# little-little-point-cloud-group/buildingSegment

Measured on AMD Instinct MI355X. Metric: Mpoints/s segmented (kNN+normal+label), higher is better.
Workload: dtype int32 coordinates / f64 normals; 1 GPU; urban_50m; points_per_gpu=50000000, k=16, max_nn=50, rg_mode=0, largest_plane=135921, seed_attempts=6951, fallback_queries=0, rg_rounds=25, validation_rejects=2, tie_rows=971975, parallelism=1 GPU, whole path

## Files before the change

### buildingsegment_amd/csrc/bs_grow_spec.hip

```cpp
#include <hipcub/hipcub.hpp>

#include <algorithm>
#include <cstdio>
#include <cstdlib>
#include <type_traits>
#include <chrono>
#include <vector>

#include "bs_centerdiv.h"
#include "bs_common.h"

namespace bs {

namespace {

constexpr int32_t INF = 0x7fffffff;
constexpr int32_t LOWER_BIT = (int32_t)0x80000000;
constexpr int32_t POS_MASK = 0x7fffffff;
constexpr int MAX_WAVES = 1 << 18;
constexpr int MAX_PENDING = 32768;

enum : int32_t { ST_NONE = 0, ST_DONE = 1, ST_FAILED0 = 2, ST_NOMEM = 3, ST_WATCHDOG = 4, ST_STOLEN = 5 };

struct SpecArgs {
// ... 188 lines not shown
    lcnt[d] = 0;
  __syncthreads();
  const uint32_t m0 = i < n ? hmask[i] : 0u;
  const uint32_t lm0 = i < n ? lmask[i] : 0u;
  const int32_t* row = rows + (i < n ? i : 0) * row_stride;
  for (uint32_t m = m0; m;) {
    const int t = __ffs(m) - 1;
    m &= m - 1;
    const int64_t d = (int64_t)row[t + 1] - w0;
    if (d >= 0 && d < RW_WIN)
      atomicAdd(&lcnt[d], 1);
  }
  __syncthreads();
  for (int d = threadIdx.x; d < RW_WIN; d += 256) {
    const int v = lcnt[d];
    if (v) {
      lbase[d] = atomicAdd(&rcur[w0 + d], (unsigned long long)v);
      lcnt[d] = 0;
    }
  }
  __syncthreads();
  for (uint32_t m = m0; m;) {
    const int t = __ffs(m) - 1;
    m &= m - 1;
    const int32_t c = row[t + 1];
    const int64_t d = (int64_t)c - w0;
    if (d >= 0 && d < RW_WIN)
      radj[lbase[d] + (unsigned)atomicAdd(&lcnt[d], 1)] = (int32_t)i | (((lm0 >> t) & 1u) ? LOWER_BIT : 0);
    else
      radj[atomicAdd(&rcur[c], 1ull)] = (int32_t)i | (((lm0 >> t) & 1u) ? LOWER_BIT : 0);
  }
}

__global__ void pull_pass_kernel(int64_t n, int K, int sub, const uint32_t* __restrict__ hmask,
                                 const int32_t* __restrict__ prio, const uint8_t* __restrict__ ps,
                                 const int32_t* __restrict__ base, const int64_t* __restrict__ roff,
                                 const int32_t* __restrict__ radj, int32_t* __restrict__ omega, uint32_t* occ,
                                 uint8_t* dirty_cur, uint8_t* dirty_next, uint8_t* bdirty_cur, uint8_t* bdirty_next,
                                 int4* rec, int quads, int* any, const int32_t* __restrict__ minr, const int* prev_any)
{
  if (prev_any && *prev_any == 0)
    return;
  __shared__ unsigned long long sub_mask;
  const int64_t nb256 = (n + 255) >> 8;
  const int64_t g0 = (int64_t)blockIdx.x * sub;
  if (threadIdx.x < 64) {
    const int64_t gidx = g0 + threadIdx.x;
    const bool d = (int)threadIdx.x < sub && gidx < nb256 && bdirty_cur[gidx] != 0;
    if (d)
      bdirty_cur[gidx] = 0;
    const unsigned long long m = ballot64(d);
    if (threadIdx.x == 0)
      sub_mask = m;
  }
  __syncthreads();
  unsigned long long gm = sub_mask;
  bool flipped = false;
  while (gm) {
    const int t = __ffsll(gm) - 1;
    gm &= gm - 1;
    const int64_t c = ((g0 + t) << 8) + threadIdx.x;
    if (c >= n || !dirty_cur[c])
      continue;
    dirty_cur[c] = 0;
    int32_t v = base[c];
    if (v > minr[c]) {
      const int64_t e1 = roff[c + 1];
      for (int64_t e = roff[c]; e < e1; e += 4) {
        int32_t j[4];
        uint32_t ow[4];
        int32_t pj[4];
#pragma unroll
        for (int i = 0; i < 4; i++)
          j[i] = e + i < e1 ? (radj[e + i] & POS_MASK) : -1;
#pragma unroll
        for (int i = 0; i < 4; i++)
          ow[i] = j[i] >= 0 ? __hip_atomic_load(occ + (j[i] >> 5), __ATOMIC_RELAXED, __HIP_MEMORY_SCOPE_AGENT) : 0u;
#pragma unroll
        for (int i = 0; i < 4; i++)
          pj[i] = ((ow[i] >> (j[i] & 31)) & 1u) ? prio[j[i]] : INF;
#pragma unroll
        for (int i = 0; i < 4; i++)
          v = pj[i] < v ? pj[i] : v;
      }
    }
    omega[c] = v;
    reinterpret_cast<int32_t*>(rec + c * quads)[3] = v;
    const uint32_t m0 = hmask[c];
    const uint8_t want = (m0 != 0 && !(ps[c] & 1) && v >= prio[c]) ? 1 : 0;
    const uint32_t cbit = 1u << (c & 31);
    const uint8_t have = (__hip_atomic_load(occ + (c >> 5), __ATOMIC_RELAXED, __HIP_MEMORY_SCOPE_AGENT) & cbit) ? 1 : 0;
    if (want != have) {
      if (want)
        __hip_atomic_fetch_or(occ + (c >> 5), cbit, __ATOMIC_RELAXED, __HIP_MEMORY_SCOPE_AGENT);
      else
        __hip_atomic_fetch_and(occ + (c >> 5), ~cbit, __ATOMIC_RELAXED, __HIP_MEMORY_SCOPE_AGENT);
      const int32_t* row = reinterpret_cast<const int32_t*>(rec + c * quads + 4);
      uint32_t m = m0;
      while (m) {
        const int b = __ffs(m) - 1;
        m &= m - 1;
        const int32_t q = row[b + 1];
        dirty_next[q] = 1;
        bdirty_next[q >> 8] = 1;
      }
      flipped = true;
    }
  }
  if (flipped)
    *any = 1;
}

__global__ void decide_init_kernel(const uint32_t* __restrict__ hmask, int64_t n, uint8_t* __restrict__ st,
                                   uint8_t* __restrict__ bund)
{
  const int64_t c = blockIdx.x * (int64_t)blockDim.x + threadIdx.x;
  const bool maker = c < n && hmask[c] != 0;
  if (c < n)
    st[c] = maker ? 0 : 2;
  const int anym = __syncthreads_or(maker);
  if (threadIdx.x == 0)
    bund[blockIdx.x] = anym ? 1 : 0;
}

__global__ void decide_pass_kernel(int64_t n, int sub, const int32_t* __restrict__ prio,
                                   const int64_t* __restrict__ roff, const int32_t* __restrict__ radj, uint8_t* st,
                                   uint8_t* bund, int* any)
{
  __shared__ unsigned long long sub_mask;
  __shared__ int left[64];
  const int64_t nb256 = (n + 255) >> 8;
  const int64_t g0 = (int64_t)blockIdx.x * sub;
  if (threadIdx.x < 64) {
    const int64_t gidx = g0 + threadIdx.x;
    const bool d = (int)threadIdx.x < sub && gidx < nb256 && bund[gidx] != 0;
    left[threadIdx.x] = 0;
    const unsigned long long m = ballot64(d);
    if (threadIdx.x == 0)
      sub_mask = m;
  }
  __syncthreads();
  unsigned long long gm = sub_mask;
  bool undecided_left = false;
  while (gm) {
    const int t = __ffsll(gm) - 1;
    gm &= gm - 1;
    const int64_t c = ((g0 + t) << 8) + threadIdx.x;
    bool mine_left = false;
    if (c < n && __hip_atomic_load(st + c, __ATOMIC_RELAXED, __HIP_MEMORY_SCOPE_AGENT) == 0) {
      bool lower_occ = false, lower_und = false;
      const int64_t e1 = roff[c + 1];
      for (int64_t e = roff[c]; e < e1; e += 4) {
        int32_t rj[4];
        uint8_t sj[4];
#pragma unroll
        for (int q = 0; q < 4; q++)
          rj[q] = e + q < e1 ? radj[e + q] : 0;
#pragma unroll
        for (int q = 0; q < 4; q++)
          sj[q] = rj[q] < 0 ? __hip_atomic_load(st + (rj[q] & POS_MASK), __ATOMIC_RELAXED, __HIP_MEMORY_SCOPE_AGENT) : (uint8_t)2;
#pragma unroll
// ... 82 lines not shown

__global__ void cand_flag_kernel(const int4* __restrict__ rec, int quads, int K,
                                 int64_t n, int32_t F, const int32_t* __restrict__ prio, const uint8_t* __restrict__ ps,
                                 int all_seeds, const int32_t* __restrict__ omega, int32_t* min_idx,
                                 unsigned long long* __restrict__ cand_out, int32_t* cand_count, uint8_t* __restrict__ bcand,
                                 int sub)
{
  __shared__ unsigned long long sub_mask;
  const int64_t nb256 = (n + 255) >> 8;
  const int64_t g0 = (int64_t)blockIdx.x * sub;
  if (threadIdx.x < 64) {
    const int64_t gidx = g0 + threadIdx.x;
    const bool live = (int)threadIdx.x < sub && gidx < nb256 && bcand[gidx] != 0;
    const unsigned long long m = ballot64(live);
    if (threadIdx.x == 0)
      sub_mask = m;
  }
  __syncthreads();
  unsigned long long gm = sub_mask;
  while (gm) {
    const int t = __ffsll(gm) - 1;
    gm &= gm - 1;
    const int64_t i = ((g0 + t) << 8) + threadIdx.x;
    bool c = false, alive = false;
    const uint8_t f = i < n ? ps[i] : (uint8_t)2;
    int32_t pi = 0;
    if (!(f & 2)) {
      pi = prio[i];
      const int32_t oi = omega[i];
      alive = !(oi < F);
      if (pi >= F && oi >= pi && (all_seeds || !(f & 1))) {
        c = true;
        const int32_t* row = reinterpret_cast<const int32_t*>(rec + i * quads + 4);
        for (int u = 1; u < K; u += 4) {
          int32_t ov[4];
#pragma unroll
          for (int q = 0; q < 4; q++)
            ov[q] = u + q < K ? omega[row[u + q]] : INF;
#pragma unroll
          for (int q = 0; q < 4; q++)
            c = c && ov[q] >= pi;
        }
      }
    }
    const int any_alive = __syncthreads_or(alive);
    if (threadIdx.x == 0 && !any_alive)
      bcand[g0 + t] = 0;
    if (c && min_idx)
      atomicMin(min_idx, pi);
    if (c && cand_out)
      cand_out[atomicAdd(cand_count, 1)] = ((unsigned long long)(uint32_t)pi << 32) | (uint32_t)i;
  }
}

template <int KC>
struct RecLayout {
  static constexpr int QUADS = 4 + KC / 4;
};

__device__ inline int32_t* rec_tag(int4* rec, int quads, int64_t i)
{
  return reinterpret_cast<int32_t*>(rec + i * quads + 2) + 2;
}

__global__ void invert_order_kernel(const int32_t* __restrict__ order, int64_t n, int32_t* __restrict__ pos)
{
  const int64_t s = blockIdx.x * (int64_t)blockDim.x + threadIdx.x;
  if (s < n)
    pos[order[s]] = (int32_t)s;
}

template <int KC>
__global__ __launch_bounds__(256) void build_records_kernel(SpecArgs a, const int32_t* __restrict__ order, const int32_t* __restrict__ pos,
// ... 1469 lines not shown
  gc = bs_grow_counters{};
  int retry_max_list = RETRY_MAX_LIST;
  bool retry_env = false;
  if (const char* e = getenv("BS_RETRY_MAX_LIST")) {
    retry_max_list = atoi(e);
    retry_env = true;
  }
  if (lim.retry_max_list >= 0) {
    retry_max_list = lim.retry_max_list;
    retry_env = true;
  }
  int retry_big_round = 1024;
  if (const char* e = getenv("BS_RETRY_BIG_ROUND"))
    retry_big_round = atoi(e);
  if (lim.retry_big_round >= 0)
    retry_big_round = lim.retry_big_round;
  int max_waves = MAX_WAVES;
  if (const char* e = getenv("BS_MAX_WAVES"))
    max_waves = atoi(e);
  if (lim.max_waves > 0)
    max_waves = (int)std::min<int64_t>(lim.max_waves, MAX_WAVES);
  const int wave_cap = (int)std::max<int64_t>(1, std::min<int64_t>(MAX_WAVES, n / 8 + 64));
  max_waves = (int)std::max<int64_t>(1, std::min<int64_t>(max_waves, wave_cap));
  const unsigned long long pool_cap = (unsigned long long)std::max<int64_t>(
      std::min<int64_t>(64 * n, (int64_t)3 << 30), 8 * n + (int64_t)(2 * 256 + 32 * 32) * 2 * wave_cap);
  const unsigned long long pool_cap_eff = lim.pool_cap > 0 ? std::min<unsigned long long>(pool_cap, (unsigned long long)lim.pool_cap) : pool_cap;
  gc.pool_cap = (int64_t)pool_cap_eff;
  gc.max_waves_end = max_waves;
  BS_HIP(ctx, ctx->rg_list.reserve(sizeof(int32_t) * list_cap));
  BS_HIP(ctx, ctx->rg_planes.reserve(sizeof(PlaneRec) * planes_cap));
  BS_HIP(ctx, ctx->rg_stats.reserve(sizeof(GrowStats)));
  const size_t n_i32 = (size_t)(7 * n + planes_cap + 1024 + 128);
  const size_t nb256 = (size_t)((n + 255) / 256);
  const size_t aux_bytes = sizeof(int32_t) * n_i32 + (size_t)5 * n + 3 * nb256 + 8192 +
                           sizeof(PlaneOut) * ((size_t)wave_cap + MAX_PENDING) +
                           sizeof(CopyDesc) * ((size_t)wave_cap + MAX_PENDING);
  BS_HIP(ctx, ctx->rg_aux.reserve(aux_bytes));
  BS_HIP(ctx, ctx->rg_stack.reserve(sizeof(int32_t) * pool_cap));
  BS_HIP(ctx, ctx->rg_radj.reserve(sizeof(int32_t) * (size_t)(n * (K - 1) + 16)));
  BS_HIP(ctx, ctx->rg_roff.reserve(sizeof(int64_t) * (size_t)(n + 2)));
  int64_t* roff = ctx->rg_roff.as<int64_t>();
  int32_t* aux = ctx->rg_aux.as<int32_t>();
  int32_t* d_misc = aux;
  uint32_t* hmask = (uint32_t*)(aux + 1024);
  int32_t* omega = aux + 1024 + n;
  int32_t* base = aux + 1024 + 2 * n;
  int32_t* dead = aux + 1024 + 3 * n;
  int32_t* prio = aux + 1024 + 4 * n;
  int32_t* rpos = aux + 1024 + 5 * n;
  int32_t* vmark = aux + 1024 + 6 * n + 64;
  int32_t* d_seeds = aux + 1024 + 7 * n + 64;
  uint8_t* flags = (uint8_t*)(aux + n_i32);
  uint8_t* ps = flags + n;
  uint32_t* occ = (uint32_t*)(((uintptr_t)(ps + n) + 15) & ~(uintptr_t)15);
  uint8_t* dirty0 = (uint8_t*)occ + ((n + 31) / 32) * 4 + 16;
  uint8_t* dirty1 = dirty0 + n;
  uint8_t* bdirty0 = dirty1 + n;
  uint8_t* bdirty1 = bdirty0 + nb256;
  uint8_t* bcand = bdirty1 + nb256;
  PlaneOut* d_out = (PlaneOut*)(((uintptr_t)(bcand + nb256) + 255) & ~(uintptr_t)255);
  PlaneOut* d_pend = d_out + wave_cap;
  CopyDesc* d_copy = (CopyDesc*)(d_pend + MAX_PENDING);
  int32_t* radj = ctx->rg_radj.as<int32_t>();
  unsigned long long* d_pool_top = (unsigned long long*)(d_misc + 16);
  Pool pool = {ctx->rg_stack.as<int32_t>(), d_pool_top, pool_cap_eff};

  SpecArgs a;
  a.xyz = d_xyz;
  a.normals = d_normals;
  a.neigh = d_neigh;
  a.n = n;
  a.K = K;
  a.th = (double)p.th_thickness;
  a.cos_th = p.cos_th;
  a.th_count = p.th_point_count;
  a.F = 0;
  a.pad = 0;

  const int KC = K <= 16 ? 16 : 32;
  const int quads = 4 + KC / 4;
  BS_HIP(ctx, ctx->rg_rec.reserve(sizeof(int4) * (size_t)quads * n));
  int4* rec = ctx->rg_rec.as<int4>();
  BS_HIP(ctx, ctx->rg_geo.reserve(sizeof(unsigned long long) * 2 * (size_t)(n + 64)));
  unsigned long long* cand_raw = ctx->rg_geo.as<unsigned long long>();
  BS_HIP(ctx, ctx->rg_gs.reserve(sizeof(int4) * 3 * (size_t)(n + 1)));
  int4* gs = ctx->rg_gs.as<int4>();
  unsigned long long* d_cand = cand_raw + n + 64;
  const size_t nt1 = (size_t)(n >> TILE1) + 2, nt2 = (size_t)(n >> TILE2) + 2;
  BS_HIP(ctx, ctx->rg_disp.reserve(sizeof(unsigned long long) * (nt1 + nt2) + sizeof(uint32_t) * 2 * (size_t)wave_cap + 64 +
                                    sizeof(PlaneOut) * (size_t)wave_cap));
  unsigned long long* tmin1 = ctx->rg_disp.as<unsigned long long>();
  unsigned long long* tmin2 = tmin1 + nt1;
  uint32_t* dkeys_in = reinterpret_cast<uint32_t*>(tmin2 + nt2);
// ... 16 lines not shown
  }
  const int4* spts_in = npos ? ctx->spts.as<int4>() : nullptr;
  const double* pnorm_in = (npos && ctx->npos_normals == d_normals) ? pnorm_of(ctx->seg_npos.as<int32_t>(), n, K) : nullptr;
  if (order && !npos) {
    pos = vmark;
    invert_order_kernel<<<nblk(n, 256), 256, 0, st>>>(order, n, pos);
  }
  if (KC == 16)
    build_records_kernel<16><<<nblk(n, 256), 256, 0, st>>>(a, order, pos, npos, rec, prio, gs, spts_in, pnorm_in);
  else
    build_records_kernel<32><<<nblk(n, 256), 256, 0, st>>>(a, order, pos, npos, rec, prio, gs, spts_in, pnorm_in);
  BS_HIP(ctx, hipMemsetAsync(rpos, 0, sizeof(int32_t) * (n + 1), st));
  uint32_t* lmask = reinterpret_cast<uint32_t*>(vmark);
  const int32_t* rows = npos ? npos : reinterpret_cast<const int32_t*>(rec) + 16;
  const int row_stride = npos ? K : quads * 4;
  static_mask_kernel<<<xcd_grid(nblk(n, 256)), 256, 0, st>>>(a, rows, row_stride, gs, hmask, rpos, lmask);
  {
    hipcub::TransformInputIterator<int64_t, ToI64, const int32_t*> in(rpos, ToI64());
    size_t tb = 0;
    BS_HIP(ctx, hipcub::DeviceScan::ExclusiveScan(nullptr, tb, in, roff, hipcub::Sum(), (int64_t)0, (int)(n + 1), st));
    BS_HIP(ctx, ctx->cub_tmp.reserve(tb));
    BS_HIP(ctx, hipcub::DeviceScan::ExclusiveScan(ctx->cub_tmp.p, tb, in, roff, hipcub::Sum(), (int64_t)0, (int)(n + 1), st));
  }
  unsigned long long* rcur = cand_raw;
  BS_HIP(ctx, hipMemcpyAsync(rcur, roff, sizeof(int64_t) * n, hipMemcpyDeviceToDevice, st));
  rev_fill_kernel<<<xcd_grid(nblk(n, 256)), 256, 0, st>>>(hmask, rows, row_stride, n, rcur, radj, lmask);
  fill_i32_kernel<<<nblk(n, 256), 256, 0, st>>>(base, n, INF);
  seed_flags_kernel<<<nblk(n, 256), 256, 0, st>>>(hmask, n, K, ps);
  BS_HIP(ctx, hipMemsetAsync(vmark, 0, sizeof(int32_t) * n, st));
  BS_HIP(ctx, hipMemsetAsync(occ, 0, sizeof(uint32_t) * (size_t)((n + 31) / 32 + 2), st));
  int64_t passes = 0;
  const int pull_sub = (int)std::max<int64_t>(1, std::min<int64_t>(64, (int64_t)nb256 / 4096));
  const int cand_sub = std::max(1, pull_sub / 8);
  {
    uint8_t* state = dirty1;
    uint8_t* bund = bdirty1;
    decide_init_kernel<<<nblk(n, 256), 256, 0, st>>>(hmask, n, state, bund);
    for (int it = 0;; it++) {
      BS_HIP(ctx, hipMemsetAsync(d_misc, 0, sizeof(int), st));
      decide_pass_kernel<<<(int)((nb256 + pull_sub - 1) / pull_sub), 256, 0, st>>>(n, pull_sub, prio, roff, radj, state, bund,
                                                                                  d_misc);
      int any = 0;
      BS_HIP(ctx, hipMemcpyAsync(&any, d_misc, sizeof any, hipMemcpyDeviceToHost, st));
      BS_HIP(ctx, hipStreamSynchronize(st));
      passes++;
      if (!any)
        break;
      if (it > 4 * 1000 * 1000)
        return fail(ctx, BS_ERR_INTERNAL, "orphan fixed point (decided states) did not converge");
    }
    decide_finish_kernel<<<nblk(n, 256), 256, 0, st>>>(n, prio, roff, radj, state, omega, occ, rec, quads, rpos);
  }
  BS_HIP(ctx, hipMemsetAsync(dirty0, 0, n, st));
  BS_HIP(ctx, hipMemsetAsync(dirty1, 0, n, st));
  BS_HIP(ctx, hipMemsetAsync(bdirty0, 0, nb256, st));
  BS_HIP(ctx, hipMemsetAsync(bdirty1, 0, nb256, st));
  BS_HIP(ctx, hipMemsetAsync(bcand, 1, nb256, st));
  BS_HIP(ctx, hipMemsetAsync(dead, 0, sizeof(int32_t) * n, st));
  uint8_t* dcur = dirty0;
  uint8_t* dnext = dirty1;
  uint8_t* bcur = bdirty0;
  uint8_t* bnext = bdirty1;
  BS_HIP(ctx, ctx->rg_hout.reserve(sizeof(PlaneOut) * ((size_t)wave_cap + MAX_PENDING) + 256));
  PlaneOut* const h_out = ctx->rg_hout.as<PlaneOut>();
  PlaneOut* const h_pend = h_out + wave_cap;
  int32_t* const h_flags = reinterpret_cast<int32_t*>(h_pend + MAX_PENDING);
  constexpr int PULL_GROUP = 16;
  int32_t* const d_flip = d_misc + 32;
  int32_t* const h_flip = h_flags + 32;
  auto propagate = [&]() -> int {
    for (int it = 0; it < 1000000; it++) {
      BS_HIP(ctx, hipMemsetAsync(d_flip, 0, sizeof(int32_t) * PULL_GROUP, st));
      for (int g = 0; g < PULL_GROUP; g++) {
        pull_pass_kernel<<<(int)((nb256 + pull_sub - 1) / pull_sub), 256, 0, st>>>(n, K, pull_sub, hmask, prio, ps, base, roff, radj,
                                                                                  omega, occ, dcur, dnext, bcur, bnext, rec, quads,
                                                                                  d_flip + g, rpos ,
                                                                                  g ? d_flip + g - 1 : nullptr);
        passes++;
        std::swap(dcur, dnext);
        std::swap(bcur, bnext);
      }
      BS_HIP(ctx, hipMemcpyAsync(h_flip, d_flip, sizeof(int32_t) * PULL_GROUP, hipMemcpyDeviceToHost, st));
      BS_HIP(ctx, hipStreamSynchronize(st));
      if (!h_flip[PULL_GROUP - 1]) {
        if (getenv("BS_VERIFY")) {
          BS_HIP(ctx, hipMemsetAsync(d_misc + 3, 0, sizeof(int), st));
          verify_fixpoint_kernel<<<nblk(n, 256), 256, 0, st>>>(n, hmask, prio, ps, base, roff, radj, omega, occ, d_misc + 3);
          int nb = 0;
          BS_HIP(ctx, hipMemcpyAsync(&nb, d_misc + 3, sizeof nb, hipMemcpyDeviceToHost, st));
          BS_HIP(ctx, hipStreamSynchronize(st));
          if (nb)
            fprintf(stderr, "[bs] VERIFY: owner structure is not a fixed point at %d points (pass %ld)\n", nb, (long)passes);
        }
        return BS_OK;
      }
    }
    return fail(ctx, BS_ERR_INTERNAL, "orphan fixed point did not converge");
  };
  int rc = propagate();
  if (rc != BS_OK)
    return rc;
  (void)hipEventRecord(ctx->ev[9], st);

  const int64_t pstore_cap = 6 * n + 65536;
  BS_HIP(ctx, ctx->rg_pstore.reserve(sizeof(int32_t) * pstore_cap));
  const int64_t pstore_lim = lim.pstore_cap > 0 ? std::min<int64_t>(pstore_cap, lim.pstore_cap) : pstore_cap;
  const int pend_lim = lim.max_pending > 0 ? (int)std::min<int64_t>(MAX_PENDING, lim.max_pending) : MAX_PENDING;
  int32_t* pstore = ctx->rg_pstore.as<int32_t>();
  int64_t pstore_top = 0;
  std::vector<PlaneOut> pending;

  std::vector<PlaneRec> recs;
  std::vector<int32_t> seeds;
  std::vector<CopyDesc> copies;
  int64_t list_used = 0, largest = 0, attempts = 0, rounds = 0, grow_launches = 0;
  double grow_ms = 0.0;
  bool timed_round = false;
// ... 26 lines not shown
  auto flush_copies = [&]() -> int {
    for (size_t off = 0; off < copies.size(); off += (size_t)wave_cap + MAX_PENDING) {
      const int nd = (int)std::min<size_t>(copies.size() - off, (size_t)wave_cap + MAX_PENDING);
      BS_HIP(ctx, hipMemcpyAsync(d_copy, copies.data() + off, sizeof(CopyDesc) * nd, hipMemcpyHostToDevice, st));
      copy_lists_kernel<<<dim3(nd, 8), 256, 0, st>>>(d_copy, nd);
      BS_HIP(ctx, hipStreamSynchronize(st));
    }
    copies.clear();
    return BS_OK;
  };
  bool cand_listed = false;
  int32_t ncand_all = 0;
  bool v3_pending = false;
  struct SideGuard {
    bs_ctx* c;
    bool* pending;
    ~SideGuard()
    {
      if (*pending && c->side)
        (void)hipStreamSynchronize(c->side);
    }
  } side_guard{ctx, &v3_pending};
  bool dead_dirty = false;
  if (!ctx->side) {
    BS_HIP(ctx, hipStreamCreateWithFlags(&ctx->side, hipStreamNonBlocking));
    BS_HIP(ctx, hipEventCreateWithFlags(&ctx->sev[0], hipEventDisableTiming));
    BS_HIP(ctx, hipEventCreateWithFlags(&ctx->sev[1], hipEventDisableTiming));
  }
  int32_t rejects_seen = 0;
  int refused_rounds = 0;
  int64_t incons[3] = {0, 0, 0};
  int forge_mode = ctx->forge_mode;
  ctx->forge_mode = 0;
  const bool dbg = getenv("BS_DEBUG") != nullptr;
  const bool do_validate3 = getenv("BS_NO_VALIDATE3") == nullptr;
  const bool use_spec2 = KC == 16 && !(getenv("BS_GROW_V2") && atoi(getenv("BS_GROW_V2")) == 0);
  auto launch_grow = [&](int cnt, const unsigned long long* cd, PlaneOut* o, int rml, const uint32_t* ord) {
    const int64_t cap = 512 * n + 4096;
    if (use_spec2)
      grow_spec2_kernel<16><<<cnt, 64, 0, st>>>(a, cd, cnt, rec, dead, pool, o, cap, rml, ord);
    else if (KC == 16)
      grow_spec_kernel<16><<<cnt, 64, 0, st>>>(a, cd, cnt, rec, dead, pool, o, cap, rml, ord);
    else
      grow_spec_kernel<32><<<cnt, 64, 0, st>>>(a, cd, cnt, rec, dead, pool, o, cap, rml, ord);
  };
  BS_HIP(ctx, hipMemsetAsync(d_misc + 4, 0, 12 * sizeof(int), st));
  for (;;) {
    rounds++;
    gc.rounds = rounds;
    a.F = F;
    const int npend = (int)pending.size();
    if (!cand_listed) {
      BS_HIP(ctx, hipMemsetAsync(d_misc + 1, 0, sizeof(int32_t), st));
      cand_flag_kernel<<<(int)((nb256 + cand_sub - 1) / cand_sub), 256, 0, st>>>(rec, quads, K, n, F, prio, ps, 0, omega, nullptr, cand_raw, d_misc + 1, bcand, cand_sub);
      BS_HIP(ctx, hipMemcpyAsync(h_flags + 11, d_misc + 1, sizeof(int32_t), hipMemcpyDeviceToHost, st));
      BS_HIP(ctx, hipStreamSynchronize(st));
      ncand_all = h_flags[11];
    }
    cand_listed = false;
    if (ncand_all == 0 && npend == 0)
      break;
    if (ncand_all > 0) {
      size_t tb = 0;
      BS_HIP(ctx, hipcub::DeviceRadixSort::SortKeys(nullptr, tb, cand_raw, d_cand, ncand_all, 0, 64, st));
      BS_HIP(ctx, ctx->cub_tmp.reserve(tb));
      BS_HIP(ctx, hipcub::DeviceRadixSort::SortKeys(ctx->cub_tmp.p, tb, cand_raw, d_cand, ncand_all, 0, 64, st));
    }
// ... 24 lines not shown
      const uint32_t* d_order = nullptr;
      if (dispatch_order && ncand >= 4096) {
        BS_HIP(ctx, hipMemsetAsync(tmin1, 0xff, sizeof(unsigned long long) * (nt1 + nt2), st));
        tile_min_kernel<<<nblk(ncand, 256), 256, 0, st>>>(d_cand, ncand, tmin1, tmin2);
        dispatch_key_kernel<<<nblk(ncand, 256), 256, 0, st>>>(d_cand, ncand, tmin1, tmin2, dkeys_in);
        size_t tb = 0;
        BS_HIP(ctx, hipcub::DeviceRadixSort::SortKeys(nullptr, tb, dkeys_in, dkeys_out, ncand, 0, 20, st));
        BS_HIP(ctx, ctx->cub_tmp.reserve(tb));
        BS_HIP(ctx, hipcub::DeviceRadixSort::SortKeys(ctx->cub_tmp.p, tb, dkeys_in, dkeys_out, ncand, 0, 20, st));
        d_order = dkeys_out;
      }
      (void)hipEventRecord(ctx->ev[6], st);
      const int rml = (ncand >= retry_big_round && !retry_env) ? 0x7fffffff : retry_max_list;
      launch_grow(ncand, d_cand, d_out, rml, d_order);
      (void)hipEventRecord(ctx->ev[7], st);
      grow_launches++;
      timed_round = true;
      if (forge_mode) {
        forge_kernel<<<1, 64, 0, st>>>(d_out, ncand, pool.base, forge_mode, d_misc + 5);
        forge_mode = 0;
      }
      validate1_kernel<<<ncand, VT, 0, st>>>(d_out, ncand, pool.base, rec, quads, dead, n, vmark,
                                             (int32_t)((rounds & 0x3ff) << 20), d_misc + 4);
      if (do_validate3) {
        BS_HIP(ctx, hipEventRecord(ctx->sev[0], st));
        BS_HIP(ctx, hipStreamWaitEvent(ctx->side, ctx->sev[0], 0));
        validate3_kernel<<<ncand, V3T, 0, ctx->side>>>(d_out, ncand, pool.base, rec, quads, d_misc + 4);
        BS_HIP(ctx, hipEventRecord(ctx->sev[1], ctx->side));
        v3_pending = true;
      }
      reset_tags_kernel<<<ncand, VT, 0, st>>>(d_out, ncand, pool.base, rec, quads, K);
      reset_dead_kernel<<<nblk(ncand, 256), 256, 0, st>>>(d_cand, ncand, dead);
      plane_apply_kernel<<<ncand, VT, 0, st>>>(d_out, ncand, pool.base, base, ps, dcur, bcur, omega, occ, rec, quads);
      rc = propagate();
      if (rc != BS_OK)
        return rc;
      validate2_kernel<<<ncand, VT, 0, st>>>(d_out, ncand, pool.base, omega, rec, quads, K);
    }
    if (npend)
      validate2_kernel<<<npend, VT, 0, st>>>(d_pend, npend, pstore, omega, rec, quads, K);
    const int32_t init2[2] = {0, INF};
    BS_HIP(ctx, hipMemcpyAsync(d_misc + 1, init2, sizeof init2, hipMemcpyHostToDevice, st));
    cand_flag_kernel<<<(int)((nb256 + cand_sub - 1) / cand_sub), 256, 0, st>>>(rec, quads, K, n, F, prio, ps, 0, omega, d_misc + 2, cand_raw, d_misc + 1, bcand, cand_sub);
    BS_HIP(ctx, hipMemcpyAsync(h_flags + 8, d_misc + 1, 2 * sizeof(int32_t), hipMemcpyDeviceToHost, st));
    if (v3_pending) {
      BS_HIP(ctx, hipStreamWaitEvent(st, ctx->sev[1], 0));
      v3_pending = false;
    }
    BS_HIP(ctx, hipMemcpyAsync(h_flags + 10, d_misc + 4, sizeof(int32_t), hipMemcpyDeviceToHost, st));
    const bool compact = ncand >= 4096 && !dbg;
    int nh = ncand;
    PlaneOut* d_outh = d_out;
    if (compact) {
      size_t tb = 0;
      BS_HIP(ctx, hipcub::DeviceSelect::If(nullptr, tb, d_out, d_outc, d_misc + 20, ncand, KeepForHost(), st));
      BS_HIP(ctx, ctx->cub_tmp.reserve(tb));
      BS_HIP(ctx, hipcub::DeviceSelect::If(ctx->cub_tmp.p, tb, d_out, d_outc, d_misc + 20, ncand, KeepForHost(), st));
      BS_HIP(ctx, hipMemcpyAsync(h_flags + 14, d_misc + 20, sizeof(int32_t), hipMemcpyDeviceToHost, st));
      BS_HIP(ctx, hipStreamSynchronize(st));
      nh = h_flags[14];
      d_outh = d_outc;
    }
    if (nh)
      BS_HIP(ctx, hipMemcpyAsync(h_out, d_outh, sizeof(PlaneOut) * nh, hipMemcpyDeviceToHost, st));
    if (npend)
      BS_HIP(ctx, hipMemcpyAsync(h_pend, d_pend, sizeof(PlaneOut) * npend, hipMemcpyDeviceToHost, st));
// ... 156 lines not shown
          rc = commit_plane(o, src);
          if (rc != BS_OK)
            return rc;
        } else if (take_p) {
          next_pending.push_back(o);
        } else if (pend_room > 0 && pstore_top + o.list_n + o.log_n + 8 <= pstore_lim) {
          pend_room--;
          PlaneOut q = o;
          q.list_off = pstore_top;
          copies.push_back({pool.base + o.list_off, pstore + q.list_off, o.list_n, nullptr});
          pstore_top += (o.list_n + 3) & ~(int64_t)3;
          q.log_off = pstore_top;
          if (o.log_n)
            copies.push_back({pool.base + o.log_off, pstore + q.log_off, o.log_n, nullptr});
          pstore_top += (o.log_n + 3) & ~(int64_t)3;
          next_pending.push_back(q);
        } else {
          o.pad = 2;
          dropped++;
          if (pend_room > 0)
            gc.dropped_pend_store++;
          else
            gc.dropped_pend_count++;
        }
      }
    }
    rc = flush_copies();
    if (rc != BS_OK)
      return rc;
    if (dropped) {
      if (nh) {
        BS_HIP(ctx, hipMemcpyAsync(d_outh, h_out, sizeof(PlaneOut) * nh, hipMemcpyHostToDevice, st));
        plane_apply_kernel<<<nh, VT, 0, st>>>(d_outh, nh, pool.base, base, ps, dcur, bcur, omega, occ, rec, quads);
      }
      if (npend) {
        BS_HIP(ctx, hipMemcpyAsync(d_pend, h_pend, sizeof(PlaneOut) * npend, hipMemcpyHostToDevice, st));
        plane_apply_kernel<<<npend, VT, 0, st>>>(d_pend, npend, pstore, base, ps, dcur, bcur, omega, occ, rec, quads);
      }
      rc = propagate();
      if (rc != BS_OK)
        return rc;
    } else {
      cand_listed = true;
      ncand_all = next_ncand_all;
    }
    pending.swap(next_pending);
    if (pending.empty())
      pstore_top = 0;
    if (first_bad == INF)
      break;
    const bool refused = rejects_now > rejects_seen;
    rejects_seen = rejects_now;
    refused_rounds = refused ? refused_rounds + 1 : 0;
    if (finals == 0 && dropped == 0 && !nomem_lowest && first_bad <= F && (!refused || refused_rounds > 8))
      return fail(ctx, BS_ERR_INTERNAL, refused ? "region grow (speculative): the validation keeps refusing a plane"
                                                : "region grow (speculative): no progress");
    F = first_bad;
    if (rounds > 4 * n + 16)
      return fail(ctx, BS_ERR_INTERNAL, "region grow (speculative): round limit");
  }
  int32_t* owner_final = omega;
  const int np = (int)recs.size();
  if (np > 0) {
    BS_HIP(ctx, hipMemcpyAsync(d_seeds, seeds.data(), sizeof(int32_t) * np, hipMemcpyHostToDevice, st));
    BS_HIP(ctx, hipMemcpyAsync(ctx->rg_planes.p, recs.data(), sizeof(PlaneRec) * np, hipMemcpyHostToDevice, st));
  }
  label_kernel<<<nblk(n, 256), 256, 0, st>>>(owner_final, n, d_seeds, np, prio, d_plane_idx);
  int32_t vstat[12] = {0};
  BS_HIP(ctx, hipMemcpyAsync(vstat, d_misc + 4, sizeof vstat, hipMemcpyDeviceToHost, st));
  GrowStats hs;
// ... 136 lines not shown
```

Baseline: 186.9 Mpoints/s.

## Drive owner propagation passes from a compacted dirty-group worklist

Replaces the full-grid scan of dirty 256-point groups in the owner fixed-point propagation with a compacted worklist. A compaction kernel builds the initial list, and each pull pass appends newly dirtied groups to the next list using wave-level staging and deduplication flags. The decide fixed-point loop is also batched into groups of passes with early-exit chaining, which cuts host syncs, and the neighbor gather loops are unrolled to 16. This adds atomics, extra buffers and a triple-buffered counter scheme, and a fixed grid of up to 4096 blocks processes the list in contiguous chunks, which may balance load poorly.

```diff
diff --git a/buildingsegment_amd/csrc/bs_grow_spec.hip b/buildingsegment_amd/csrc/bs_grow_spec.hip
--- a/buildingsegment_amd/csrc/bs_grow_spec.hip
+++ b/buildingsegment_amd/csrc/bs_grow_spec.hip
@@ -244,12 +244,154 @@
   }
 }
 
+constexpr int OWN_TRIP = 16;
+constexpr int WL_CAP = 1024;
+constexpr int WL_WAVE = 256;
+
+__device__ __forceinline__ void wl_flush(const int* l_buf, int* l_base, int staged, int32_t* list, int* cnt)
+{
+  if (threadIdx.x == 0)
+    *l_base = atomicAdd(cnt, staged);
+  __syncthreads();
+  const int b = *l_base;
+  for (int i = threadIdx.x; i < staged; i += blockDim.x)
+    list[b + i] = l_buf[i];
+  __syncthreads();
+}
+
+__global__ __launch_bounds__(256) void wl_compact_kernel(uint8_t* bdirty, int nb, uint32_t* gflag, int32_t* list, int* cnt)
+{
+  __shared__ int l_buf[WL_CAP];
+  __shared__ int l_base;
+  __shared__ int wsum[4];
+  int staged = 0;
+  for (int j = 0; j < WL_CAP / 256; j++) {
+    const int g = blockIdx.x * WL_CAP + j * 256 + threadIdx.x;
+    bool add = false;
+    if (g < nb && bdirty[g]) {
+      bdirty[g] = 0;
+      add = atomicExch(gflag + g, 1u) == 0u;
+    }
+    const unsigned long long am = ballot64(add);
+    if ((threadIdx.x & 63) == 0)
+      wsum[threadIdx.x >> 6] = __popcll(am);
+    __syncthreads();
+    int before = __popcll(am & ((1ull << (threadIdx.x & 63)) - 1ull)), total = 0;
+    for (int w = 0; w < 4; w++) {
+      before += w < (int)(threadIdx.x >> 6) ? wsum[w] : 0;
+      total += wsum[w];
+    }
+    if (add)
+      l_buf[staged + before] = g;
+    staged += total;
+    __syncthreads();
+  }
+  if (staged)
+    wl_flush(l_buf, &l_base, staged, list, cnt);
+}
+
+__device__ __forceinline__ void wl_wave_flush(int* wbuf, int& staged, int32_t* list, int* cnt)
+{
+  const int lane = threadIdx.x & 63;
+  __builtin_amdgcn_fence(__ATOMIC_RELEASE, "workgroup");
+  __builtin_amdgcn_wave_barrier();
+  int b = 0;
+  if (lane == 0)
+    b = atomicAdd(cnt, staged);
+  b = __shfl(b, 0);
+  for (int i = lane; i < staged; i += 64)
+    list[b + i] = wbuf[i];
+  __builtin_amdgcn_fence(__ATOMIC_ACQ_REL, "workgroup");
+  __builtin_amdgcn_wave_barrier();
+  staged = 0;
+}
+
+__device__ __forceinline__ void wl_add(bool want, int32_t g, uint32_t* gflag, int* wbuf, int& staged, int32_t* list, int* cnt)
+{
+  if (!ballot64(want))
+    return;
+  const bool added = want && atomicExch(gflag + g, 1u) == 0u;
+  const unsigned long long am = ballot64(added);
+  if (am == 0)
+    return;
+  if (added)
+    wbuf[staged + __popcll(am & ((1ull << (threadIdx.x & 63)) - 1ull))] = g;
+  staged += __popcll(am);
+  if (staged > WL_WAVE - 64)
+    wl_wave_flush(wbuf, staged, list, cnt);
+}
+
+struct PullEval {
+  bool flip;
+  bool walked;
+  uint32_t m0;
+};
+
+__device__ __forceinline__ PullEval pull_eval(int64_t c, const uint32_t* __restrict__ hmask, const int32_t* __restrict__ prio,
+                                              const uint8_t* __restrict__ ps, const int32_t* __restrict__ base,
+                                              const int64_t* __restrict__ roff, const int32_t* __restrict__ radj,
+                                              int32_t* __restrict__ omega, uint32_t* occ, int4* rec, int quads,
+                                              const int32_t* __restrict__ minr)
+{
+  int32_t v = base[c];
+  const int32_t mr = minr[c];
+  const int64_t e0 = roff[c], e1 = roff[c + 1];
+  const uint32_t m0 = hmask[c];
+  const uint8_t psc = ps[c];
+  const int32_t pc = prio[c];
+  const uint32_t cbit = 1u << (c & 31);
+  const uint32_t oword = __hip_atomic_load(occ + (c >> 5), __ATOMIC_RELAXED, __HIP_MEMORY_SCOPE_AGENT);
+  const bool walk = v > mr;
+  if (walk) {
+    for (int64_t e = e0; e < e1; e += OWN_TRIP) {
+      int32_t j[OWN_TRIP];
+      uint32_t ow[OWN_TRIP];
+      int32_t pj[OWN_TRIP];
+#pragma unroll
+      for (int i = 0; i < OWN_TRIP; i++)
+        j[i] = radj[e + i < e1 ? e + i : e1 - 1] & POS_MASK;
+#pragma unroll
+      for (int i = 0; i < OWN_TRIP; i++)
+        ow[i] = __hip_atomic_load(occ + (j[i] >> 5), __ATOMIC_RELAXED, __HIP_MEMORY_SCOPE_AGENT);
+#pragma unroll
+      for (int i = 0; i < OWN_TRIP; i++) {
+        const bool o = ((ow[i] >> (j[i] & 31)) & 1u) != 0;
+        pj[i] = prio[o ? (int64_t)j[i] : c];
+        pj[i] = o ? pj[i] : INF;
+      }
+#pragma unroll
+      for (int i = 0; i < OWN_TRIP; i++)
+        v = pj[i] < v ? pj[i] : v;
+    }
+  }
+  omega[c] = v;
+  reinterpret_cast<int32_t*>(rec + c * quads)[3] = v;
+  const bool want = m0 != 0 && !(psc & 1) && v >= pc;
+  const bool have = (oword & cbit) != 0;
+  if (want != have) {
+    if (want)
+      __hip_atomic_fetch_or(occ + (c >> 5), cbit, __ATOMIC_RELAXED, __HIP_MEMORY_SCOPE_AGENT);
+    else
+      __hip_atomic_fetch_and(occ + (c >> 5), ~cbit, __ATOMIC_RELAXED, __HIP_MEMORY_SCOPE_AGENT);
+  }
+  return {want != have, walk, m0};
+}
+
+__device__ __forceinline__ void pull_stats(int* dbg, bool dirty, bool walked)
+{
+  const int nd = __popcll(ballot64(dirty)), nw = __popcll(ballot64(walked));
+  if ((threadIdx.x & 63) == 0 && nd) {
+    atomicAdd(dbg + 1, nd);
+    atomicAdd(dbg + 2, nw);
+  }
+}
+
 __global__ void pull_pass_kernel(int64_t n, int K, int sub, const uint32_t* __restrict__ hmask,
                                  const int32_t* __restrict__ prio, const uint8_t* __restrict__ ps,
                                  const int32_t* __restrict__ base, const int64_t* __restrict__ roff,
                                  const int32_t* __restrict__ radj, int32_t* __restrict__ omega, uint32_t* occ,
                                  uint8_t* dirty_cur, uint8_t* dirty_next, uint8_t* bdirty_cur, uint8_t* bdirty_next,
-                                 int4* rec, int quads, int* any, const int32_t* __restrict__ minr, const int* prev_any)
+                                 int4* rec, int quads, int* any, const int32_t* __restrict__ minr, const int* prev_any, int* dbg)
 {
   if (prev_any && *prev_any == 0)
     return;
@@ -267,48 +409,26 @@
   }
   __syncthreads();
   unsigned long long gm = sub_mask;
+  if (dbg && threadIdx.x == 0 && gm) {
+    atomicAdd(dbg, __popcll(gm));
+    atomicMax(dbg + 3, __popcll(gm));
+  }
   bool flipped = false;
   while (gm) {
     const int t = __ffsll(gm) - 1;
     gm &= gm - 1;
     const int64_t c = ((g0 + t) << 8) + threadIdx.x;
-    if (c >= n || !dirty_cur[c])
-      continue;
-    dirty_cur[c] = 0;
-    int32_t v = base[c];
-    if (v > minr[c]) {
-      const int64_t e1 = roff[c + 1];
-      for (int64_t e = roff[c]; e < e1; e += 4) {
-        int32_t j[4];
-        uint32_t ow[4];
-        int32_t pj[4];
-#pragma unroll
-        for (int i = 0; i < 4; i++)
-          j[i] = e + i < e1 ? (radj[e + i] & POS_MASK) : -1;
-#pragma unroll
-        for (int i = 0; i < 4; i++)
-          ow[i] = j[i] >= 0 ? __hip_atomic_load(occ + (j[i] >> 5), __ATOMIC_RELAXED, __HIP_MEMORY_SCOPE_AGENT) : 0u;
-#pragma unroll
-        for (int i = 0; i < 4; i++)
-          pj[i] = ((ow[i] >> (j[i] & 31)) & 1u) ? prio[j[i]] : INF;
-#pragma unroll
-        for (int i = 0; i < 4; i++)
-          v = pj[i] < v ? pj[i] : v;
-      }
-    }
-    omega[c] = v;
-    reinterpret_cast<int32_t*>(rec + c * quads)[3] = v;
-    const uint32_t m0 = hmask[c];
-    const uint8_t want = (m0 != 0 && !(ps[c] & 1) && v >= prio[c]) ? 1 : 0;
-    const uint32_t cbit = 1u << (c & 31);
-    const uint8_t have = (__hip_atomic_load(occ + (c >> 5), __ATOMIC_RELAXED, __HIP_MEMORY_SCOPE_AGENT) & cbit) ? 1 : 0;
-    if (want != have) {
-      if (want)
-        __hip_atomic_fetch_or(occ + (c >> 5), cbit, __ATOMIC_RELAXED, __HIP_MEMORY_SCOPE_AGENT);
-      else
-        __hip_atomic_fetch_and(occ + (c >> 5), ~cbit, __ATOMIC_RELAXED, __HIP_MEMORY_SCOPE_AGENT);
+    const bool d = c < n && dirty_cur[c] != 0;
+    PullEval r = {false, false, 0u};
+    if (d) {
+      dirty_cur[c] = 0;
+      r = pull_eval(c, hmask, prio, ps, base, roff, radj, omega, occ, rec, quads, minr);
+    }
+    if (dbg)
+      pull_stats(dbg, d, r.walked);
+    if (r.flip) {
       const int32_t* row = reinterpret_cast<const int32_t*>(rec + c * quads + 4);
-      uint32_t m = m0;
+      uint32_t m = r.m0;
       while (m) {
         const int b = __ffs(m) - 1;
         m &= m - 1;
@@ -319,6 +439,86 @@
       flipped = true;
     }
   }
+  if (flipped)
+    *any = 1;
+}
+
+__global__ __launch_bounds__(256) void pull_list_kernel(int64_t n, int K, const uint32_t* __restrict__ hmask,
+                                                        const int32_t* __restrict__ prio, const uint8_t* __restrict__ ps,
+                                                        const int32_t* __restrict__ base, const int64_t* __restrict__ roff,
+                                                        const int32_t* __restrict__ radj, int32_t* __restrict__ omega,
+                                                        uint32_t* occ, uint8_t* dirty_cur, uint8_t* dirty_next,
+                                                        const int32_t* __restrict__ list_cur, int32_t* list_next,
+                                                        uint32_t* gflag_cur, uint32_t* gflag_next, int* cnt, int s_cur,
+                                                        int s_nxt, int s_clr, int4* rec, int quads, int* any,
+                                                        const int32_t* __restrict__ minr, int* dbg)
+{
+  __shared__ int l_buf[4][WL_WAVE];
+  int* const wbuf = l_buf[threadIdx.x >> 6];
+  const int lane = threadIdx.x & 63;
+  const int ncur = cnt[s_cur];
+  if (blockIdx.x == 0 && threadIdx.x == 0) {
+    cnt[s_clr] = 0;
+    if (dbg && ncur) {
+      dbg[0] = ncur;
+      dbg[3] = (ncur + (int)gridDim.x - 1) / (int)gridDim.x;
+    }
+  }
+  if (ncur == 0)
+    return;
+  int staged = 0;
+  bool flipped = false;
+  const int per = (ncur + (int)gridDim.x - 1) / (int)gridDim.x;
+  const int i0 = blockIdx.x * per, i1 = min(ncur, i0 + per);
+  if (i0 >= i1)
+    return;
+  int32_t g_next = list_cur[i0];
+  for (int idx = i0; idx < i1; idx++) {
+    const int32_t g = g_next;
+    if (idx + 1 < i1)
+      g_next = list_cur[idx + 1];
+    const int64_t c = ((int64_t)g << 8) + threadIdx.x;
+    if (threadIdx.x == 0)
+      gflag_cur[g] = 0;
+    const bool d = c < n && dirty_cur[c] != 0;
+    PullEval r = {false, false, 0u};
+    if (d) {
+      dirty_cur[c] = 0;
+      r = pull_eval(c, hmask, prio, ps, base, roff, radj, omega, occ, rec, quads, minr);
+    }
+    if (dbg)
+      pull_stats(dbg, d, r.walked);
+    if (!ballot64(r.flip))
+      continue;
+    flipped = flipped || r.flip;
+    const int32_t* row = reinterpret_cast<const int32_t*>(rec + (d ? c : 0) * quads + 4);
+    for (int b0 = 0; b0 + 1 < K; b0 += OWN_TRIP) {
+      int32_t gq[OWN_TRIP];
+      uint32_t fl[OWN_TRIP];
+      bool rep[OWN_TRIP];
+#pragma unroll
+      for (int i = 0; i < OWN_TRIP; i++) {
+        const int b = b0 + i;
+        gq[i] = -1;
+        if (r.flip && b + 1 < K && ((r.m0 >> b) & 1u)) {
+          const int32_t q = row[b + 1];
+          dirty_next[q] = 1;
+          gq[i] = q >> 8;
+        }
+      }
+#pragma unroll
+      for (int i = 0; i < OWN_TRIP; i++) {
+        const int32_t left = __shfl_up(gq[i], 1);
+        rep[i] = gq[i] >= 0 && (lane == 0 || left != gq[i]) && (i == 0 || gq[i - 1] != gq[i]);
+        fl[i] = __hip_atomic_load(gflag_next + (rep[i] ? gq[i] : g), __ATOMIC_RELAXED, __HIP_MEMORY_SCOPE_AGENT);
+      }
+#pragma unroll
+      for (int i = 0; i < OWN_TRIP; i++)
+        wl_add(rep[i] && fl[i] == 0u, gq[i], gflag_next, wbuf, staged, list_next, cnt + s_nxt);
+    }
+  }
+  if (staged)
+    wl_wave_flush(wbuf, staged, list_next, cnt + s_nxt);
   if (flipped)
     *any = 1;
 }
@@ -337,8 +537,10 @@
 
 __global__ void decide_pass_kernel(int64_t n, int sub, const int32_t* __restrict__ prio,
                                    const int64_t* __restrict__ roff, const int32_t* __restrict__ radj, uint8_t* st,
-                                   uint8_t* bund, int* any)
-{
+                                   uint8_t* bund, int* any, const int* prev_any)
+{
+  if (prev_any && *prev_any == 0)
+    return;
   __shared__ unsigned long long sub_mask;
   __shared__ int left[64];
   const int64_t nb256 = (n + 255) >> 8;
@@ -487,13 +689,17 @@
       if (pi >= F && oi >= pi && (all_seeds || !(f & 1))) {
         c = true;
         const int32_t* row = reinterpret_cast<const int32_t*>(rec + i * quads + 4);
-        for (int u = 1; u < K; u += 4) {
-          int32_t ov[4];
+        for (int u = 1; u < K; u += OWN_TRIP) {
+          int32_t nb[OWN_TRIP];
+          int32_t ov[OWN_TRIP];
 #pragma unroll
-          for (int q = 0; q < 4; q++)
-            ov[q] = u + q < K ? omega[row[u + q]] : INF;
+          for (int q = 0; q < OWN_TRIP; q++)
+            nb[q] = row[u + q < K ? u + q : K - 1];
 #pragma unroll
-          for (int q = 0; q < 4; q++)
+          for (int q = 0; q < OWN_TRIP; q++)
+            ov[q] = omega[nb[q]];
+#pragma unroll
+          for (int q = 0; q < OWN_TRIP; q++)
             c = c && ov[q] >= pi;
         }
       }
@@ -2029,7 +2235,7 @@
   BS_HIP(ctx, ctx->rg_stats.reserve(sizeof(GrowStats)));
   const size_t n_i32 = (size_t)(7 * n + planes_cap + 1024 + 128);
   const size_t nb256 = (size_t)((n + 255) / 256);
-  const size_t aux_bytes = sizeof(int32_t) * n_i32 + (size_t)5 * n + 3 * nb256 + 8192 +
+  const size_t aux_bytes = sizeof(int32_t) * n_i32 + (size_t)5 * n + 3 * nb256 + 16 * nb256 + 8192 +
                            sizeof(PlaneOut) * ((size_t)wave_cap + MAX_PENDING) +
                            sizeof(CopyDesc) * ((size_t)wave_cap + MAX_PENDING);
   BS_HIP(ctx, ctx->rg_aux.reserve(aux_bytes));
@@ -2055,7 +2261,13 @@
   uint8_t* bdirty0 = dirty1 + n;
   uint8_t* bdirty1 = bdirty0 + nb256;
   uint8_t* bcand = bdirty1 + nb256;
-  PlaneOut* d_out = (PlaneOut*)(((uintptr_t)(bcand + nb256) + 255) & ~(uintptr_t)255);
+  int32_t* wl_list[2];
+  uint32_t* wl_flag[2];
+  wl_list[0] = (int32_t*)(((uintptr_t)(bcand + nb256) + 15) & ~(uintptr_t)15);
+  wl_list[1] = wl_list[0] + nb256;
+  wl_flag[0] = (uint32_t*)(wl_list[1] + nb256);
+  wl_flag[1] = wl_flag[0] + nb256;
+  PlaneOut* d_out = (PlaneOut*)(((uintptr_t)(wl_flag[1] + nb256) + 255) & ~(uintptr_t)255);
   PlaneOut* d_pend = d_out + wave_cap;
   CopyDesc* d_copy = (CopyDesc*)(d_pend + MAX_PENDING);
   int32_t* radj = ctx->rg_radj.as<int32_t>();
@@ -2138,24 +2350,43 @@
   int64_t passes = 0;
   const int pull_sub = (int)std::max<int64_t>(1, std::min<int64_t>(64, (int64_t)nb256 / 4096));
   const int cand_sub = std::max(1, pull_sub / 8);
+  const bool use_wl = !(getenv("BS_OWNER_WORKLIST") && atoi(getenv("BS_OWNER_WORKLIST")) == 0);
+  int own_grid = (int)std::min<size_t>(nb256, 4096);
+  if (const char* e = getenv("BS_OWNER_GRID"))
+    own_grid = std::max(1, std::min(own_grid, atoi(e)));
+  constexpr int PULL_GROUP = 16;
+  int own_group = PULL_GROUP;
+  if (const char* e = getenv("BS_OWNER_GROUP"))
+    own_group = std::max(2, std::min(PULL_GROUP, atoi(e)));
+  int* const wl_cnt = d_misc + 64;
+  int64_t wl_pass = 0;
+  bool wl_marked = false;
+  const bool dbg = getenv("BS_DEBUG") != nullptr;
+  BS_HIP(ctx, ctx->rg_hout.reserve(sizeof(PlaneOut) * ((size_t)wave_cap + MAX_PENDING) + 256));
+  PlaneOut* const h_out = ctx->rg_hout.as<PlaneOut>();
+  PlaneOut* const h_pend = h_out + wave_cap;
+  int32_t* const h_flags = reinterpret_cast<int32_t*>(h_pend + MAX_PENDING);
+  int32_t* const h_cnt = h_flags + 48;
   {
     uint8_t* state = dirty1;
     uint8_t* bund = bdirty1;
+    int32_t* const d_any = d_misc + 32;
     decide_init_kernel<<<nblk(n, 256), 256, 0, st>>>(hmask, n, state, bund);
     for (int it = 0;; it++) {
-      BS_HIP(ctx, hipMemsetAsync(d_misc, 0, sizeof(int), st));
-      decide_pass_kernel<<<(int)((nb256 + pull_sub - 1) / pull_sub), 256, 0, st>>>(n, pull_sub, prio, roff, radj, state, bund,
-                                                                                  d_misc);
-      int any = 0;
-      BS_HIP(ctx, hipMemcpyAsync(&any, d_misc, sizeof any, hipMemcpyDeviceToHost, st));
+      BS_HIP(ctx, hipMemsetAsync(d_any, 0, sizeof(int32_t) * PULL_GROUP, st));
+      for (int g = 0; g < own_group; g++, passes++)
+        decide_pass_kernel<<<(int)((nb256 + pull_sub - 1) / pull_sub), 256, 0, st>>>(n, pull_sub, prio, roff, radj, state, bund,
+                                                                                    d_any + g, g ? d_any + g - 1 : nullptr);
+      BS_HIP(ctx, hipMemcpyAsync(h_cnt, d_any + own_group - 1, sizeof(int32_t), hipMemcpyDeviceToHost, st));
       BS_HIP(ctx, hipStreamSynchronize(st));
-      passes++;
-      if (!any)
+      if (h_cnt[0] == 0)
         break;
       if (it > 4 * 1000 * 1000)
         return fail(ctx, BS_ERR_INTERNAL, "orphan fixed point (decided states) did not converge");
     }
     decide_finish_kernel<<<nblk(n, 256), 256, 0, st>>>(n, prio, roff, radj, state, omega, occ, rec, quads, rpos);
+    BS_HIP(ctx, hipMemsetAsync(wl_cnt, 0, 3 * sizeof(int), st));
+    BS_HIP(ctx, hipMemsetAsync(wl_flag[0], 0, sizeof(uint32_t) * 2 * nb256, st));
   }
   BS_HIP(ctx, hipMemsetAsync(dirty0, 0, n, st));
   BS_HIP(ctx, hipMemsetAsync(dirty1, 0, n, st));
@@ -2167,28 +2398,49 @@
   uint8_t* dnext = dirty1;
   uint8_t* bcur = bdirty0;
   uint8_t* bnext = bdirty1;
-  BS_HIP(ctx, ctx->rg_hout.reserve(sizeof(PlaneOut) * ((size_t)wave_cap + MAX_PENDING) + 256));
-  PlaneOut* const h_out = ctx->rg_hout.as<PlaneOut>();
-  PlaneOut* const h_pend = h_out + wave_cap;
-  int32_t* const h_flags = reinterpret_cast<int32_t*>(h_pend + MAX_PENDING);
-  constexpr int PULL_GROUP = 16;
   int32_t* const d_flip = d_misc + 32;
   int32_t* const h_flip = h_flags + 32;
+  int32_t* const d_pstat = d_misc + 128;
   auto propagate = [&]() -> int {
+    if (use_wl && wl_marked)
+      wl_compact_kernel<<<(int)((nb256 + WL_CAP - 1) / WL_CAP), 256, 0, st>>>(bcur, (int)nb256, wl_flag[wl_pass & 1], wl_list[wl_pass & 1],
+                                                                      wl_cnt + wl_pass % 3);
+    wl_marked = false;
     for (int it = 0; it < 1000000; it++) {
       BS_HIP(ctx, hipMemsetAsync(d_flip, 0, sizeof(int32_t) * PULL_GROUP, st));
-      for (int g = 0; g < PULL_GROUP; g++) {
-        pull_pass_kernel<<<(int)((nb256 + pull_sub - 1) / pull_sub), 256, 0, st>>>(n, K, pull_sub, hmask, prio, ps, base, roff, radj,
-                                                                                  omega, occ, dcur, dnext, bcur, bnext, rec, quads,
-                                                                                  d_flip + g, rpos ,
-                                                                                  g ? d_flip + g - 1 : nullptr);
+      if (dbg)
+        BS_HIP(ctx, hipMemsetAsync(d_pstat, 0, sizeof(int32_t) * 4 * PULL_GROUP, st));
+      for (int g = 0; g < own_group; g++) {
+        if (use_wl) {
+          const int cur = (int)(wl_pass & 1);
+          pull_list_kernel<<<own_grid, 256, 0, st>>>(n, K, hmask, prio, ps, base, roff, radj, omega, occ, dcur, dnext, wl_list[cur],
+                                                    wl_list[cur ^ 1], wl_flag[cur], wl_flag[cur ^ 1], wl_cnt, (int)(wl_pass % 3),
+                                                    (int)((wl_pass + 1) % 3), (int)((wl_pass + 2) % 3), rec, quads, d_flip + g,
+                                                    rpos , dbg ? d_pstat + 4 * g : nullptr);
+          wl_pass++;
+        } else {
+          pull_pass_kernel<<<(int)((nb256 + pull_sub - 1) / pull_sub), 256, 0, st>>>(n, K, pull_sub, hmask, prio, ps, base, roff, radj,
+                                                                                    omega, occ, dcur, dnext, bcur, bnext, rec, quads,
+                                                                                    d_flip + g, rpos ,
+                                                                                    g ? d_flip + g - 1 : nullptr,
+                                                                                    dbg ? d_pstat + 4 * g : nullptr);
+        }
         passes++;
         std::swap(dcur, dnext);
         std::swap(bcur, bnext);
       }
       BS_HIP(ctx, hipMemcpyAsync(h_flip, d_flip, sizeof(int32_t) * PULL_GROUP, hipMemcpyDeviceToHost, st));
+      if (dbg) {
+        int32_t hs[4 * PULL_GROUP];
+        BS_HIP(ctx, hipMemcpyAsync(hs, d_pstat, sizeof hs, hipMemcpyDeviceToHost, st));
+        BS_HIP(ctx, hipStreamSynchronize(st));
+        for (int g = 0; g < own_group; g++)
+          if (hs[4 * g])
+            fprintf(stderr, "[bs] owner pass %ld: dirty groups %d, dirty points %d, walked their list %d, most groups in one workgroup %d\n",
+                    (long)(passes - own_group + g), hs[4 * g], hs[4 * g + 1], hs[4 * g + 2], hs[4 * g + 3]);
+      }
       BS_HIP(ctx, hipStreamSynchronize(st));
-      if (!h_flip[PULL_GROUP - 1]) {
+      if (!h_flip[own_group - 1]) {
         if (getenv("BS_VERIFY")) {
           BS_HIP(ctx, hipMemsetAsync(d_misc + 3, 0, sizeof(int), st));
           verify_fixpoint_kernel<<<nblk(n, 256), 256, 0, st>>>(n, hmask, prio, ps, base, roff, radj, omega, occ, d_misc + 3);
@@ -2281,7 +2533,6 @@
   int64_t incons[3] = {0, 0, 0};
   int forge_mode = ctx->forge_mode;
   ctx->forge_mode = 0;
-  const bool dbg = getenv("BS_DEBUG") != nullptr;
   const bool do_validate3 = getenv("BS_NO_VALIDATE3") == nullptr;
   const bool use_spec2 = KC == 16 && !(getenv("BS_GROW_V2") && atoi(getenv("BS_GROW_V2")) == 0);
   auto launch_grow = [&](int cnt, const unsigned long long* cd, PlaneOut* o, int rml, const uint32_t* ord) {
@@ -2372,6 +2623,7 @@
       reset_tags_kernel<<<ncand, VT, 0, st>>>(d_out, ncand, pool.base, rec, quads, K);
       reset_dead_kernel<<<nblk(ncand, 256), 256, 0, st>>>(d_cand, ncand, dead);
       plane_apply_kernel<<<ncand, VT, 0, st>>>(d_out, ncand, pool.base, base, ps, dcur, bcur, omega, occ, rec, quads);
+      wl_marked = true;
       rc = propagate();
       if (rc != BS_OK)
         return rc;
@@ -2594,10 +2846,12 @@
       if (nh) {
         BS_HIP(ctx, hipMemcpyAsync(d_outh, h_out, sizeof(PlaneOut) * nh, hipMemcpyHostToDevice, st));
         plane_apply_kernel<<<nh, VT, 0, st>>>(d_outh, nh, pool.base, base, ps, dcur, bcur, omega, occ, rec, quads);
+        wl_marked = true;
       }
       if (npend) {
         BS_HIP(ctx, hipMemcpyAsync(d_pend, h_pend, sizeof(PlaneOut) * npend, hipMemcpyHostToDevice, st));
         plane_apply_kernel<<<npend, VT, 0, st>>>(d_pend, npend, pstore, base, ps, dcur, bcur, omega, occ, rec, quads);
+        wl_marked = true;
       }
       rc = propagate();
       if (rc != BS_OK)
```

Result: faster. 197.9 Mpoints/s, median of 6 (+5.9%).
